# Amelie-Schreiber/ShapeMol

Hardware: AMD Instinct MI355X
Metric: molecules/sec (1000-step DDPM sample, batch 256) (higher is better)
Workload: dtype f32 (matrix operands split exactly into 3 x bf16 pieces = 24 bits, six piece products, fp32 accumulate); 1 GPU; BASELINE configs[1]: batch 256 MOSES-prior molecules (9-27 atoms) per GPU, 1000-step chain, fp32 results, k=8, synthetic shapes + hash-filled weights; besides the 5 warm-up steps an untimed 200-step chain runs first to reach the loaded clocks; batch_per_gpu=256, atoms_per_gpu=5541, total_atoms=5541, noise=device Philox, trajectories=kept in HBM, launch=hipGraph replay, parallelism=dp1 (whole batches per rank), ranks_seen=1

## Files before the change

### shapemol_amd/csrc/shapemol_hip.hip

```cpp
#include "../../include/shapemol_hip.h"
#include "sm_device.h"
#include "sm_edge.h"
#include "sm_edge_bf16.h"
#include "sm_edge16.h"
#include "sm_node.h"
#include "sm_node16.h"
#include "sm_edge_stream.h"
#include "sm_misc.h"
#include "sm_cfg.h"
#include "sm_guide_groups.h"
#include "sm_mesh.h"
#include <hip/hip_ext.h>

#include <algorithm>
#include <cmath>
#include <cstdio>
#include <cstring>
#include <map>
#include <string>
#include <type_traits>
#include <vector>

#include "sm_pack.h"
#include "sm_devmem.h"
// ... 82 lines not shown
    int num_cu = 256;
    CloudSet cs; MeshSet ms; DevList mem_cs, mem_ms;
    int2 *wg_table = nullptr; int64_t wg_table_cap = 0; DevList mem_wg;
    shapemol_sd_ctx *field_sd = nullptr; double field_lr = 0.0; int field_step = 0;
    float4 *m_within = nullptr; int *m_out = nullptr, *m_cnt = nullptr; int64_t m_cap = 0, m_cnt_cap = 0; DevList mem_mesh;
    int64_t m_flag_groups = 0;
    double cfg_w = 0.0, cfg_p = 0.0; int cfg_type = 0, cfg_has_bounds = 0; float cfg_lo[3] = {}, cfg_hi[3] = {};
    float *cfg_tr_pos_u = nullptr, *cfg_tr_v_u = nullptr;
    float *pred_pos_u = nullptr, *pred_v_u = nullptr;
    float *shape_zero = nullptr;
    float *cfg_stat = nullptr; double *cfg_part = nullptr; unsigned *cfg_hist = nullptr;
    CfgGroupSet cgs;
    int *cfg_mol_grp = nullptr; int2 *cfg_blk_tab = nullptr; double *cfg_gpart = nullptr; int64_t cfg_tab_stride = 0;
    int first_step = 0;
    int *pin_off = nullptr, *pin_atom = nullptr, *pin_nbr = nullptr; int64_t n_pins = 0; int pin_steps = 0, pin_k = 0; DevList mem_pins;
    bool prof_on = false;
    std::vector<ProfRec> prof;
    hipEvent_t cur_e0 = nullptr, cur_e1 = nullptr;
    hipGraphExec_t gexec = nullptr, gexec_u = nullptr;
    int64_t n_captures = 0;
    int64_t launch_rec[8] = {}, graph_rec[8] = {};
    int64_t node_rec[8] = {};
    int64_t x2h_out_rec[4] = {};
    struct GraphKey { int64_t N = 0, B = 0; Guide guide = Guide::None; int fold = 0, gfuse = 0;
                      int cfg = 0 ; double cfgv[9] = {};
                      int cfg_groups = 0;
                      uint64_t field_gen = 0; double field_lr = 0.0; int field_step = 0;
                      bool operator==(const GraphKey &o) const {
                          if (!(N == o.N && B == o.B && guide == o.guide && fold == o.fold && gfuse == o.gfuse && cfg == o.cfg &&
                                cfg_groups == o.cfg_groups && field_gen == o.field_gen && field_lr == o.field_lr &&
                                field_step == o.field_step)) return false;
                          for (int i = 0; i < 9; ++i) if (cfgv[i] != o.cfgv[i]) return false;
                          return true;
                      } } gkey{};
    hipStream_t gstream = nullptr; bool gstream_set = false;
    void drop_graphs() {
        if (!gexec && !gexec_u) return;
        if (!gstream_set || hipStreamSynchronize(gstream) != hipSuccess) hipDeviceSynchronize();
        if (gexec) { hipGraphExecDestroy(gexec); gexec = nullptr; }
        if (gexec_u) { hipGraphExecDestroy(gexec_u); gexec_u = nullptr; }
    }
    const float *P(size_t off) const { return d_img + off; }
};

namespace {

#define SMK(kern, grid, block, shm, stream, ...)                                                                    \
    do {                                                                                                             \
        if (c->prof_on) hipExtLaunchKernelGGL(kern, grid, block, shm, stream, c->cur_e0, c->cur_e1, 0, __VA_ARGS__); \
        else hipLaunchKernelGGL(kern, grid, block, shm, stream, __VA_ARGS__);                                        \
    } while (0)

// ... 65 lines not shown
    if (N <= c->capN && B <= c->capB) return 0;
    HIPCHK(hipSetDevice(c->device));
    HIPCHK(hipDeviceSynchronize());
    c->drop_graphs();
    const int64_t capN = std::max<int64_t>(N, c->capN), capB = std::max<int64_t>(B, c->capB);
    c->ws.release();
    c->capN = c->capB = 0; c->lastN = c->lastB = 0; c->last_h = c->last_x = nullptr;
    if (workspace_alloc(c, capN, capB)) { c->ws.release(); return 1; }
    c->capN = capN; c->capB = capB;
    return 0;
}

}

#include "sm_guide_host.h"

namespace {

constexpr int kVnFoldBytes = kVnFoldCap * 3 * 4 + 32 * 8;

template <int H>
lg::In launch_in(const shapemol_ctx *c, int n_atoms) {
    constexpr bool chain16_fits = Chain16Lds<H>::BYTES <= 2 * EdgeImage16<H, H / 16>::TOTAL * 4;
    return {c->opt, {kVnFoldCap, kStreamTPR, CHAIN_COLS, kGraphCap, kLin6Chunk, chain16_fits}, c->KP, c->num_cu, H, n_atoms};
}

#define ATTR(bytes, ...) HIPCHK(hipFuncSetAttribute((const void *)__VA_ARGS__, hipFuncAttributeMaxDynamicSharedMemorySize, (int)(bytes)))
template <int H, int K>
int set_edge_attr_k() {
    constexpr int NT = H / 16;
    constexpr int vn_tail = vn_red_doubles(12, H / 8) * 8 + 12 * 96 * 4;
    constexpr int fold = K <= 16 ? kVnFoldBytes : 0;
    constexpr int x16 = 2 * EdgeImage16<H, NT>::TOTAL * 4 + fold, h16 = (EdgeImage16<H, NT>::TOTAL + EdgeImage16<H, 1>::TOTAL) * 4 + vn_tail;
    ATTR(x16, edge16_kernel<H, K, false>); ATTR(x16, edge16_kernel<H, K, false, true>);
    ATTR(x16, edge16_loop_kernel<H, K, false>); ATTR(x16, edge16_loop_kernel<H, K, false, true>);
    ATTR(h16, edge16_kernel<H, K, true>); ATTR(h16, edge16_kernel<H, K, true, true>);
    ATTR(h16, edge16_loop_kernel<H, K, true>); ATTR(h16, edge16_loop_kernel<H, K, true, true>);
    ATTR((StreamMap<H, false>::O_TAIL * 4 + kVnFoldBytes), edge_stream_kernel<H, K, false>);
    ATTR((StreamMap<H, true>::O_TAIL * 4 + (NT + kStreamProducers) * 64 * 2 * 8), edge_stream_kernel<H, K, true>);
    if constexpr (K <= 16) {
        constexpr int xph = EdgePhaseImage<H, NT>::TOTAL * 4, hph = (EdgePhaseImage<H, NT>::TOTAL + EdgePhaseImage<H, 1>::TOTAL) * 4 + vn_tail;
        ATTR(x16, x2h_chain16_kernel<H, K>); ATTR(x16, x2h_chain16_kernel<H, K, true>);
        ATTR((EdgeBlob<H, false>::TOTAL * 4), edge_attention_kernel<H, K, false>); ATTR((EdgeBlob<H, true>::TOTAL * 4), edge_attention_kernel<H, K, true>);
        ATTR(xph, edge_fused_kernel<H, K, false, false>); ATTR(xph, edge_fused_kernel<H, K, false, true>);
        ATTR(hph, edge_fused_kernel<H, K, true, false>); ATTR(hph, edge_fused_kernel<H, K, true, true>);
    }
    return 0;
// ... 314 lines not shown
    c->tab_key = 0;
    LAUNCH("prep", SMK(prologue_tab_index_kernel, dim3((unsigned)((rows + 255) / 256)), dim3(256), 0, s, c->tab_v, c->tab_mol_of, c->tab_t_mol, c->tab_flag, T, C));
    const NodePrologueArgs pa = prologue_args<H>(c, c->tab_v, c->tab_mol_of, c->tab_t_mol, nullptr, c->etab, c->q_tab, c->pre_tab, (int)rows);
    if (launch_prologue<H>(c, s, pa, c->tab_flag)) return 1;
    c->tab_key = prologue_tab_key(c);
    return 0;
}

template <int H>
int run_score(shapemol_ctx *c, hipStream_t s, const ShapePrep &sp, const float *x_in, const int64_t *v_in, int64_t N, int64_t B,
              bool sampling, int t_first, float *out_pos, float *out_h, float *out_v, bool reuse_graph = false) {
    const shapemol_config &g = c->cfg;
    const int L = g.num_layers, hd = g.n_heads, C = g.num_classes, D = g.time_emb_dim, KP = c->KP;
    const int n = (int)N;
    AtomEmbArgs ae{c->P(c->dm.embw), c->P(c->dm.embb), v_in, c->mol_of, c->ttab, c->t_mol, sampling ? c->steps : nullptr,
                   c->steps + 1, c->bn_acc, c->h_a, n, H, C, D, t_first, L * kBnReplicas * 2 * hd + L};
    const int nlay = c->opt.stop_layer >= 0 ? std::min(c->opt.stop_layer, L) : L;
    const lg::In gi = launch_in<H>(c, n);
    const lg::StepForms sf = lg::step_forms(gi, sampling, c->n_pins > 0);
    if (sf.fused_prologue && c->opt.prologue_tab) {
        if (c->tab_key != prologue_tab_key(c)) return fail("run_score: the prologue tables are not built for this precision mode");
        PrologueTabArgs ta{c->etab, c->q_tab, c->pre_tab, c->tab_flag, v_in, c->mol_of, c->t_mol, ae.step_ptr, ae.step_cur, c->bn_acc,
                           sp.add0, c->h_a, c->q_x, c->pre0, c->status + ST_RANGE, n, C, g.num_timesteps, t_first, ae.bn_acc_len};
        LAUNCH("node_prologue", SMK(node_prologue_tab_kernel<H>, dim3((unsigned)((N * 16 + kProTabThreads - 1) / kProTabThreads)), dim3(kProTabThreads), 0, s, ta));
    } else if (sf.fused_prologue) {
        NodePrologueArgs pa = prologue_args<H>(c, v_in, c->mol_of, c->t_mol, sp.add0, c->h_a, c->q_x, c->pre0, n);
        pa.step_ptr = ae.step_ptr; pa.step_cur = ae.step_cur; pa.bn_acc = c->bn_acc; pa.bn_acc_len = ae.bn_acc_len; pa.t_first = t_first;
        if (nlay == 0) pa.n_lin_tiles = 0;
        pa.stamps = c->kstamp_sel == 5 ? c->kstamps : nullptr;
        if (launch_prologue<H>(c, s, pa)) return 1;
    } else {
        LAUNCH("embed", SMK(atom_embed_kernel, dim3((N * H + 255) / 256), dim3(256), 0, s, ae));
    }
    int64_t (&rec)[8] = c->launch_rec;
    std::fill(rec, rec + 8, 0);
    std::fill(c->node_rec, c->node_rec + 8, 0);
    std::fill(c->x2h_out_rec, c->x2h_out_rec + 4, 0);
    rec[0] = sampling; rec[1] = sf.graph_fused; rec[7] = c->num_cu;
    if (sf.stream && nlay > 0) { const lg::StreamGeom g = lg::stream_geom(gi); rec[5] = g.chunk; rec[6] = g.grid; }
    if (reuse_graph) {
    } else if (sf.graph_fused) {
        GraphArgs ga{x_in, c->mol_span, n, g.knn, KP, c->nbr, c->P(c->dm.ew.w1), c->P(c->dm.ew.b1), c->P(c->dm.ew.g), c->P(c->dm.ew.be),
                     c->P(c->dm.ew.w2), c->P(c->dm.ew.b2), c->ew, c->status + ST_SPAN, c->kstamp_sel == 4 ? c->kstamps : nullptr};
        const int apb = kGraphWaves * (KP >= 16 ? 1 : 16 / KP);
        DISPATCH_KP("graph", graph_kernel, (), dim3((n + apb - 1) / apb), dim3(kGraphWaves * 64), 0, s, ga);
    } else LAUNCH("knn", SMK(knn_kernel, dim3((N + 3) / 4), dim3(256), 0, s, x_in, c->mol_of, c->mol_off, n, g.knn, KP, c->nbr));
    if (sampling && c->n_pins > 0 && !reuse_graph)
        LAUNCH("knn", SMK(knn_pin_kernel, dim3(32), dim3(256), 0, s, c->pin_off, c->pin_steps, c->pin_atom, c->pin_nbr, c->pin_k, KP, c->steps + 1, n, c->nbr));
    EdgeWeightArgs ea{x_in, c->nbr, c->P(c->dm.ew.w1), c->P(c->dm.ew.b1), c->P(c->dm.ew.g), c->P(c->dm.ew.be),
                      c->P(c->dm.ew.w2), c->P(c->dm.ew.b2), c->ew, n * KP, KP};
    if (!sf.graph_fused && !reuse_graph) {
        const int tiles = (n * KP + 15) / 16;
        LAUNCH("edge_weight", SMK(edge_weight_kernel<H>, dim3((tiles + 3) / 4), dim3(256), 0, s, ea));
    }
    const float *cur_x = x_in;
    float *cur_h = c->h_a;
    constexpr int NT = H / 16;
    bool v_done = false;
    if (nlay > 0 && !sf.fused_prologue) {
        const DevLayer &D0 = c->dm.layer[0];
        if (launch_linear<H>(c, s, "node_pre", cur_h, c->P(D0.pre_x2h), c->P(D0.pre6_x2h), c->P(D0.pre16_x2h), sp.add0, 4 * H, c->pre0, 4 * H, 4 * NT, n,
                             c->kstamp_sel == 0 ? c->kstamps : nullptr)) return 1;
        if (launch_mlp2<H, 1>(c, s, "node_q", D0.q_x2h, cur_h, nullptr, NODE_LN_RELU, nullptr, c->q_x, H, H, n)) return 1;
    }
    double *stat_acc = c->bn_acc;
    if (c->bn_eval) {
// ... 112 lines not shown
        }
        cur_x = x_next;
    }
    c->last_h = cur_h; c->last_x = cur_x;
    if (nlay == 0 && out_pos) HIPCHK(hipMemcpyAsync(out_pos, x_in, N * 3 * sizeof(float), hipMemcpyDeviceToDevice, s));
    if (out_v && !v_done) {
        if (launch_mlp2<H, 1>(c, s, "v_head", c->dm.vhead, cur_h, nullptr, NODE_SSP, nullptr, out_v, C, C, n)) return 1;
    }
    return 0;
}

template <int H>
int run_ddpm(shapemol_ctx *c, hipStream_t s, int64_t N) {
    const shapemol_config &g = c->cfg;
    DdpmArgs a{};
    a.pred_pos = c->pred_pos; a.pred_v = c->pred_v; a.x_t = c->x_state; a.v_t = c->v_state; a.mol_of = c->mol_of;
    a.t_first = c->cfg.num_timesteps - 1;
    a.c0 = c->P(c->dm.tab[0]); a.ct = c->P(c->dm.tab[1]); a.logvar = c->P(c->dm.tab[2]); a.log_a = c->P(c->dm.tab[3]);
    a.log_1ma = c->P(c->dm.tab[4]); a.log_abar = c->P(c->dm.tab[5]); a.log_1mabar = c->P(c->dm.tab[6]);
    a.cp = c->chain_params; a.step_cur = c->steps + 1; a.step_ptr = c->steps;
    a.x_next = c->x_state; a.v_next = c->v_state;
    a.n_atoms = (int)N; a.C = g.num_classes;
    a.vf = c->ddpm_vf; c->ddpm_vf = DdpmFold{};
    const CfgArgs cfg = cfg_args(c, N);
    if (c->stamp_on) LAUNCH("stamp", SMK(clock_stamp_kernel, dim3(1), dim3(64), 0, s, c->stamps, c->steps + 1, 1024));
    if (g.num_classes <= 16) LAUNCH("ddpm", SMK(ddpm_step16_kernel, dim3((N * 16 + 255) / 256), dim3(256), 0, s, a, cfg));
    else LAUNCH("ddpm", SMK(ddpm_step_kernel<32>, dim3((N + 127) / 128), dim3(128), 0, s, a, cfg));
    return 0;
}

int check_cfg(const shapemol_config &g) {
    if (g.hidden_dim != 128 && g.hidden_dim != 32) return fail("hidden_dim must be 128 (or 32 for the reduced test model)");
    if (g.n_heads * 8 != g.hidden_dim) return fail("hidden_dim / n_heads must be 8");
    if (g.num_r_gaussian != 20) return fail("num_r_gaussian must be 20 (fixed RBF centres)");
    if (g.knn < 1 || g.knn > 32) return fail("knn must be in 1..32");
    if (g.shape_dim < 1 || g.shape_dim > 64 || g.shape_latent_dim < 4 || g.shape_latent_dim > 64 || (g.shape_latent_dim & 3))
        return fail("shape_dim must be 1..64, shape_latent_dim a multiple of 4 in 4..64");
    if (g.time_emb_dim < 4 || g.time_emb_dim > 16 || (g.time_emb_dim & 1)) return fail("time_emb_dim must be even, 4..16");
    if (g.num_classes < 2 || g.num_classes > 32) return fail("num_classes must be 2..32");
    if (g.num_layers < 1 || g.num_timesteps < 1) return fail("num_layers / num_timesteps must be positive");
    return 0;
}

template <typename F>
auto dispatch_h(const shapemol_ctx *c, F &&f) {
    return c->cfg.hidden_dim == 128 ? f(std::integral_constant<int, 128>{}) : f(std::integral_constant<int, 32>{});
}

}
// ... 65 lines not shown
        HIPCHK(c->mem_bn.alloc(&c->bn_run, 2 * count * sizeof(float)));
        HIPCHK(c->mem_bn.alloc(&c->bn_eval_acc, (size_t)L * kBnReplicas * 2 * hd * sizeof(double)));
    }
    HIPCHK(hipMemcpy(c->bn_run, h_mean, count * sizeof(float), hipMemcpyHostToDevice));
    HIPCHK(hipMemcpy(c->bn_run + count, h_var, count * sizeof(float), hipMemcpyHostToDevice));
    return 0;
}

int shapemol_reserve(shapemol_ctx *c, int64_t max_atoms, int64_t max_mols) {
    if (!c || max_atoms < 1 || max_mols < 1) return fail("shapemol_reserve: bad argument");
    return ensure_workspace(c, max_atoms, max_mols);
}

int shapemol_score(shapemol_ctx *c, const float *d_pos, const int64_t *d_v, const int64_t *d_batch, int64_t N,
                   int64_t B, const float *d_shape, const int64_t *d_t, float *out_pos, float *out_h, float *out_v,
                   void *stream) {
    if (!c || !d_pos || !d_v || !d_batch || !d_shape || !d_t || !out_pos || !out_v) return fail("shapemol_score: null argument");
    if (N < 1 || B < 1 || N > (1 << 27)) return fail("shapemol_score: n_atoms / n_mols out of range");
    HIPCHK(hipSetDevice(c->device));
    if (ensure_workspace(c, N, B)) return 1;
    hipStream_t s = (hipStream_t)stream;
    c->lastN = N; c->lastB = B;
    if (dispatch_h(c, [&](auto h) { return ensure_prologue_tables<h()>(c, s); })) return 1;
    HIPCHK(hipMemsetAsync(c->status, 0, 8 * sizeof(int), s));
    if (dispatch_h(c, [&](auto h) { return run_prep<h()>(c, s, d_batch, N, B, d_shape, c->prep[0]); })) return 1;
    LAUNCH("prep", SMK(t_convert_kernel, dim3((B + 255) / 256), dim3(256), 0, s, d_t, (int)B, c->cfg.num_timesteps, c->t_mol, c->status));
    LAUNCH("prep", SMK(v_check_kernel, dim3((N + 255) / 256), dim3(256), 0, s, d_v, (int)N, c->cfg.num_classes, c->status));
    return dispatch_h(c, [&](auto h) { return run_score<h()>(c, s, c->prep[0], d_pos, d_v, N, B, false, 0, out_pos, out_h, out_v); });
}

int shapemol_sample(shapemol_ctx *c, const float *d_init_pos, const int64_t *d_init_v, const int64_t *d_batch,
                    int64_t N, int64_t B, const float *d_shape, int32_t num_steps, const float *d_eps, const float *d_u,
                    uint64_t seed, const shapemol_traj *traj, float *out_pos, int64_t *out_v, int32_t use_graph, void *stream) {
    if (!c || !d_init_pos || !d_init_v || !d_batch || !d_shape || !out_pos || !out_v) return fail("shapemol_sample: null argument");
    if (N < 1 || B < 1 || N > (1 << 27)) return fail("shapemol_sample: n_atoms / n_mols out of range");
    if (num_steps < 1 || c->first_step + num_steps > c->cfg.num_timesteps) return fail("shapemol_sample: num_steps out of range");
    if ((d_eps == nullptr) != (d_u == nullptr)) return fail("shapemol_sample: d_eps and d_u must be given together");
    HIPCHK(hipSetDevice(c->device));
    if (ensure_workspace(c, N, B)) return 1;
    hipStream_t s = (hipStream_t)stream;
    c->lastN = N; c->lastB = B;
    if (dispatch_h(c, [&](auto h) { return ensure_prologue_tables<h()>(c, s); })) return 1;
    const int t_first = c->cfg.num_timesteps - 1;
    const Guide kind = chain_guide(c);
    const bool mesh = kind == Guide::Mesh, cfg = kind == Guide::Cfg;
    if (mesh && mesh_workspace(c, N, c->ms.groups)) return 1;
// ... 15 lines not shown
    if (cfg) {
        if (dispatch_h(c, [&](auto h) { return run_prep_shape<h()>(c, s, B, c->shape_zero, c->prep[1]); })) return 1;
        HIPCHK(hipMemsetAsync(c->cfg_hist, 0, (size_t)2 * kCfgHistWords * sizeof(unsigned), s));
        if (c->cgs.groups > 0) {
            const CfgArgs ca = cfg_args(c, N);
            HIPCHK(hipMemsetAsync(c->cgs.hist, 0, (size_t)c->cgs.groups * 2 * kCfgHistWords * sizeof(unsigned), s));
            LAUNCH("prep", SMK(cfg_groups_table_kernel, dim3(1), dim3(256), 0, s, d_batch, (int)N, ca.C, ca.n_groups, (int)B, ca.pf, c->cgs.rows,
                               c->cfg_mol_grp, c->cfg_blk_tab, ca.tab_stride, ca.blocks[0], ca.blocks[1]));
            c->cgs.stream = s; c->cgs.stream_set = true; c->cgs.last_groups = c->cgs.groups;
        }
    }
    LAUNCH("prep", SMK(v_check_kernel, dim3((N + 255) / 256), dim3(256), 0, s, d_init_v, (int)N, c->cfg.num_classes, c->status));
    {
        ChainParams cp{};
        cp.seed = seed; cp.eps = d_eps; cp.u = d_u; cp.step_base = c->first_step; cp.guide_draws = mesh ? c->ms.draws : c->cs.draws;
        if (traj) { cp.tr_pos = traj->pos_traj; cp.tr_v = traj->v_traj; cp.tr_v0 = traj->v0_traj; cp.tr_vt = traj->vt_traj;
                    cp.tr_pos_cond = traj->pos_cond_traj; cp.tr_v_cond = traj->v_cond_traj; }
        if (cfg && c->cgs.groups > 0) { cp.tr_pos_uncond = c->cgs.tr_pos_u; cp.tr_v_uncond = c->cgs.tr_v_u; }
        else if (cfg) { cp.tr_pos_uncond = c->cfg_tr_pos_u; cp.tr_v_uncond = c->cfg_tr_v_u; }
        LAUNCH("prep", SMK(set_chain_params_kernel, dim3(1), dim3(1), 0, s, c->chain_params, cp, c->steps));
    }
    HIPCHK(hipMemcpyAsync(c->x_state, d_init_pos, N * 3 * sizeof(float), hipMemcpyDeviceToDevice, s));
    HIPCHK(hipMemcpyAsync(c->v_state, d_init_v, N * sizeof(int64_t), hipMemcpyDeviceToDevice, s));
    auto one_step = [&]() -> int {
        if (dispatch_h(c, [&](auto h) { return run_score<h()>(c, s, c->prep[0], c->x_state, c->v_state, N, B, true, t_first, c->pred_pos, nullptr, c->pred_v); })) return 1;
        if (cfg) {
            if (dispatch_h(c, [&](auto h) { return run_score<h()>(c, s, c->prep[1], c->x_state, c->v_state, N, B, true, t_first, c->pred_pos_u, nullptr, c->pred_v_u, true); }) ||
                run_cfg_stats(c, s, cfg_args(c, N))) return 1;
        }
        if (enqueue_guidance(c, s, kind, c->pred_pos, N, c->steps + 1, t_first)) return 1;
        return dispatch_h(c, [&](auto h) { return run_ddpm<h()>(c, s, N); });
    };
    if (use_graph && !c->prof_on) {
        shapemol_ctx::GraphKey key{};
        const lg::StepForms sf = dispatch_h(c, [&](auto h) { return lg::step_forms(launch_in<h()>(c, (int)N), true, c->n_pins > 0); });
        key.N = N; key.B = B; key.guide = kind; key.fold = sf.fold; key.gfuse = sf.graph_fused;
        if (kind == Guide::Field) { key.field_gen = field_gen; key.field_lr = c->field_lr; key.field_step = c->field_step; }
        if (cfg && c->cgs.groups > 0) {
            key.cfg = 1 + c->cgs.type; key.cfg_groups = c->cgs.groups; key.cfgv[1] = c->cgs.p;
        } else if (cfg) {
            key.cfg = 1 + c->cfg_type;
            const double v[9] = {c->cfg_w, c->cfg_p, (double)c->cfg_has_bounds, c->cfg_lo[0], c->cfg_lo[1], c->cfg_lo[2], c->cfg_hi[0], c->cfg_hi[1], c->cfg_hi[2]};
            std::copy(v, v + 9, key.cfgv);
        }
        auto capture = [&](int n_steps, hipGraphExec_t *exec) -> int {
            hipGraph_t graph = nullptr;
            HIPCHK(hipStreamBeginCapture(s, hipStreamCaptureModeThreadLocal));
            int rc = 0;
            for (int i = 0; i < n_steps && !rc; ++i) rc = one_step();
            const hipError_t ce = hipStreamEndCapture(s, &graph);
            if (rc) { if (graph) hipGraphDestroy(graph); return 1; }
            if (ce != hipSuccess) return fail(std::string("hipStreamEndCapture: ") + hipGetErrorString(ce));
            const hipError_t ie = hipGraphInstantiate(exec, graph, nullptr, nullptr, 0);
            hipGraphDestroy(graph);
            if (ie != hipSuccess) { *exec = nullptr; return fail(std::string("hipGraphInstantiate: ") + hipGetErrorString(ie)); }
            ++c->n_captures;
            hipGraphUpload(*exec, s);
            return 0;
        };
// ... 41 lines not shown
        return 0;
    }
    if (k == "stop_layer") c->opt.stop_layer = (int)value;
    else if (k == "edge_bf16") {
        if (value < 0 || value > 3) return fail("edge_bf16 must be 0 (fp32 MFMA), 1 (exactly split bf16, phase kernels), 2 (exactly split bf16, streaming kernels) or 3 (two-piece f16)");
        if (value != 3 && value != 2 && c->KP > 16) return fail("k > 16 runs on the streaming (edge_bf16 = 2) or the two-piece f16 (edge_bf16 = 3) edge kernels");
        if (value == 3 && c->hid_max > 6.0e4f) return fail("edge_bf16 = 3: the edge MLPs' LayerNorm outputs may exceed the fp16 range for these weights");
        c->opt.edge_bf16 = (int)value;
    }
    else if (k == "edge_tiles") { if (value < -1 || value > 1) return fail("edge_tiles must be -1 (automatic), 0 (sliced one-job launches) or 1 (looping launch)"); c->opt.edge_tiles = (int)value; }
    else if (k == "node_f16") c->opt.node_f16 = value != 0;
    else if (k == "feat_f16") {
        if (value && (c->opt.edge_bf16 != 3 || !c->opt.node_f16)) return fail("feat_f16 = 1 needs the f16 kernels (edge_bf16 = 3, node_f16 = 1)");
        c->opt.feat_f16 = value != 0;
    }
    else if (k == "lin_fuse") c->opt.lin_fuse = value != 0;
    else if (k == "stream_whole_rounds") c->opt.stream_whole_rounds = value != 0;
    else if (k == "x2h_chain") c->opt.x2h_chain = value != 0;
    else if (k == "graph_fuse") c->opt.graph_fuse = value != 0;
    else if (k == "bn_eval") c->bn_eval = value != 0;
    else if (k == "ddpm_fold") c->opt.ddpm_fold = value != 0;
    else if (k == "vn_fold") c->opt.vn_fold = value != 0;
    else if (k == "prologue_tab") c->opt.prologue_tab = value != 0;
    else if (k == "lin_bf16") c->opt.lin_bf16 = (int)value;
    else if (k == "chain_bf16") c->opt.chain_bf16 = (int)value;
    else if (k == "vn_fuse") c->opt.vn_fuse = (int)value;
    else if (k == "node_levels") c->opt.node_levels = value != 0;
    else if (k == "x2h_out_fuse") { if (value < 0 || value > 2) return fail("x2h_out_fuse must be 0 (node_out6_kernel), 1 (x2h tail inside its boundary) or 2 (x2h tail always)"); c->opt.x2h_out_fuse = (int)value; }
    else if (k == "stream_chunk") { if (value < 0 || value > 4096) return fail("stream_chunk must be 0 (automatic) .. 4096"); c->opt.stream_chunk_opt = (int)value; }
    else if (k == "after_order") { if (value < 0 || value > 2) return fail("after_order must be 0 (follow-up jobs first), 1 (interleaved) or 2 (linear jobs first)"); c->opt.after_order = (int)value; }
    else if (k == "after_waves") { if (value < 1 || value > 16) return fail("after_waves must be 1..16"); c->opt.after_waves = (int)value; }
    else if (k == "after_lin_wgs") { if (value < 0 || value > 4096) return fail("after_lin_wgs must be 0 (automatic) .. 4096"); c->opt.after_lin_wgs = (int)value; }
    else if (k == "lin_waves") { if (value < 1 || value > 16) return fail("lin_waves must be 1..16"); c->opt.lin_waves = (int)value; }
    else if (k == "stamps") c->stamp_on = (int)value;
    else if (k == "kstamp_sel") c->kstamp_sel = (int)value;
    else if (k == "edge_waves") { if (value < 0 || value > 12) return fail("edge_waves must be 0 (automatic) .. 12"); c->opt.edge_threads = (int)value * 64; }
    else return fail("unknown option " + k);
    hipSetDevice(c->device);
    c->drop_graphs();
    return 0;
}

int64_t shapemol_debug_read(shapemol_ctx *c, const char *name, void *dst, size_t max_bytes) {
    if (!c || !name || !dst) { fail("shapemol_debug_read: null argument"); return -1; }
    const std::string k(name);
    const shapemol_config &g = c->cfg;
    const int64_t N = c->lastN;
    const void *src = nullptr; size_t bytes = 0;
    int64_t dims[8] = {N, c->lastB, c->KP, g.hidden_dim, g.n_heads, g.num_layers, c->capN, c->capB};
    if (k == "dims") { if (max_bytes < sizeof(dims)) return -1; std::memcpy(dst, dims, sizeof(dims)); return sizeof(dims); }
    if (k == "captures") { if (max_bytes < 8) return -1; std::memcpy(dst, &c->n_captures, 8); return 8; }
    if (k == "launch") { if (max_bytes < sizeof(c->launch_rec)) return -1; std::memcpy(dst, c->launch_rec, sizeof(c->launch_rec)); return sizeof(c->launch_rec); }
    if (k == "launch_x2h_out") { if (max_bytes < sizeof(c->x2h_out_rec)) return -1; std::memcpy(dst, c->x2h_out_rec, sizeof(c->x2h_out_rec)); return sizeof(c->x2h_out_rec); }
    if (k == "launch_node") { if (max_bytes < sizeof(c->node_rec)) return -1; std::memcpy(dst, c->node_rec, sizeof(c->node_rec)); return sizeof(c->node_rec); }
    if (k == "nbr") { src = c->nbr; bytes = N * c->KP * 4; }
    else if (k == "ew") { src = c->ew; bytes = N * c->KP * 4; }
    else if (k == "h") { src = c->last_h; bytes = N * g.hidden_dim * 4; }
    else if (k == "x") { src = c->last_x; bytes = N * 3 * 4; }
    else if (k == "h0") { src = c->h_a; bytes = N * g.hidden_dim * 4; }
    else if (k == "q_x") { src = c->q_x; bytes = N * g.hidden_dim * 4; }
    else if (k == "pre0") { src = c->pre0; bytes = N * 4 * g.hidden_dim * 4; }
    else if (k == "add0") { src = c->prep[0].add0; bytes = (size_t)c->lastB * 4 * g.hidden_dim * 4; }
    else if (k == "pre") { src = c->preAB; bytes = N * 8 * g.hidden_dim * 4; }
    else if (k == "q") { src = c->q_h; bytes = N * g.hidden_dim * 4; }
    else if (k == "att") { src = c->att; bytes = N * g.hidden_dim * 4; }
    else if (k == "o3") { src = c->o3; bytes = N * 48 * 4; }
    else if (k == "stamps") { src = c->stamps; bytes = 2048 * 8; }
    else if (k == "kstamps") { src = c->kstamps; bytes = (size_t)8 * 16 * 4096 * 8; }
    else if (k == "vn_err") { src = c->status + ST_VN_BARRIER; bytes = 4; }
    else if (k == "mesh_group_flags") { src = c->m_cnt ? c->m_cnt + 4 * c->m_cnt_cap : nullptr; bytes = (size_t)c->m_flag_groups * 4; }
    else if (k == "cfg_stat") { src = c->cfg_stat; bytes = 2 * 4; }
    else if (k == "cfg_group_stat") { src = c->cgs.last_groups > 0 ? c->cgs.stat : nullptr; bytes = (size_t)c->cgs.last_groups * 2 * 4; }
    else if (k == "bnstat") { src = c->bn_acc; bytes = (size_t)g.num_layers * kBnReplicas * 2 * g.n_heads * 8; }
    else { fail("shapemol_debug_read: unknown buffer " + k); return -1; }
    if (!src || bytes > max_bytes) { fail("shapemol_debug_read: buffer unavailable or destination too small"); return -1; }
    if (hipSetDevice(c->device) != hipSuccess || hipDeviceSynchronize() != hipSuccess ||
// ... 163 lines not shown
```

### shapemol_amd/csrc/sm_launch.h

```cpp
#pragma once
#include <algorithm>

namespace lg {

struct Options {
    int stop_layer = -1, edge_threads = 0 , lin_waves = 16, edge_bf16 = 2, lin_bf16 = 1, chain_bf16 = 1, vn_fuse = 2;
    int vn_fold = 1;
    int max_mol_atoms = 0;
    int stream_whole_rounds = 0;
    int lin_fuse = 0;
    int ddpm_fold = 1;
    int graph_fuse = 1;
    int x2h_chain = 1;
    int node_levels = 1;
    int x2h_out_fuse = 1;
    int stream_chunk_opt = 0;
    int after_order = 2;
    int after_waves = 16;
    int after_lin_wgs = 0;
    int node_f16 = 0;
    int feat_f16 = 0;
    int edge_tiles = -1;
    int prologue_tab = 1;
};

struct KernelConsts { int vn_fold_cap, stream_tpr, chain_cols, graph_cap, lin6_chunk; bool chain16_fits; };

struct In { Options o; KernelConsts k; int KP, num_cu, H, n_atoms; };

inline int cdiv(int a, int b) { return (a + b - 1) / b; }

struct Jobs { int apj, jobs; bool half; };
inline Jobs tile_jobs(int KP, int n_atoms) {
    const int apj = KP >= 16 ? 1 : 16 / KP;
    return {apj, KP > 16 ? 2 * n_atoms : cdiv(n_atoms, apj), KP > 16};
}

enum class Form { One, Loop, Sliced, Strided };
struct EdgeGeom { Form form; int apj, jobs, waves, grid, chunk, slice, atoms_per_wg; };

inline int edge_waves(const In &in, int jobs) {
    return in.o.edge_threads > 0 ? in.o.edge_threads / 64 : std::max(4, std::min(12, cdiv(jobs, in.num_cu)));
}
inline EdgeGeom one_job_geom(const In &in, int waves) {
    const Jobs j = tile_jobs(in.KP, in.n_atoms);
    const int grid = std::max(1, std::min(in.num_cu, cdiv(j.jobs, waves)));
    return {j.jobs <= grid * waves ? Form::One : Form::Strided, j.apj, j.jobs, waves, grid, waves, grid * waves, j.half ? 0 : waves * j.apj};
}

inline EdgeGeom edge_fp32_geom(const In &in) {
    const Jobs j = tile_jobs(in.KP, in.n_atoms);
// ... 68 lines not shown
    const int slots = in.num_cu * per_cu;
    g.n_fjobs = n_follow * g.n_pairs;
    g.tpg = 1;
    if (lin_tiles > 0) {
        const int ogroups = cdiv(lin_tiles, g.lw);
        const int lin_wgs = in.o.after_lin_wgs > 0 ? in.o.after_lin_wgs : std::max(slots - g.n_fjobs, slots / 2);
        g.tpg = std::max(1, cdiv(g.n_ct, std::max(1, lin_wgs / ogroups)));
        g.n_ljobs = ogroups * cdiv(g.n_ct, g.tpg);
    }
    g.lin_chunk = std::min(g.tpg, per_cu == 2 ? kAfterChunk : in.k.lin6_chunk);
    return g;
}

struct StepForms {
    bool fused_prologue;
    bool graph_fused;
    bool fold;
    bool f16, stream, phases;
    bool half_tiles;
    bool lin_fused;
    bool levels;
    bool out_fused;
    bool xc_fused;
};
inline StepForms step_forms(const In &in, bool sampling, bool pins) {
    const Options &o = in.o;
    const int KP = in.KP, m = o.max_mol_atoms;
    StepForms f{};
    f.fused_prologue = o.chain_bf16 && o.lin_bf16;
    f.graph_fused = sampling && o.graph_fuse && m > 0 && m <= in.k.graph_cap && KP <= 32 && !pins;
    f.f16 = o.edge_bf16 == 3; f.stream = o.edge_bf16 == 2; f.phases = o.edge_bf16 && KP <= 16;
    f.half_tiles = (f.f16 || f.stream) && KP > 16;
    f.lin_fused = o.chain_bf16 && o.lin_bf16 && o.node_f16 && o.lin_fuse;
    f.levels = o.node_levels && o.chain_bf16 && o.lin_bf16 && !o.node_f16 && !f.lin_fused;
    const StreamGeom sg = stream_geom(in);
    const EdgeGeom e16 = edge16_geom(in), xc = x2h_chain_geom(in);
    f.xc_fused = f.f16 && o.x2h_chain && KP <= 16 && o.chain_bf16 && o.node_f16 && !o.lin_fuse && o.edge_threads == 0 &&
                 xc.form == Form::One && xc.waves <= 12 && xc.atoms_per_wg <= in.k.chain_cols * 16 && in.k.chain16_fits;
    f.out_fused = f.stream && o.x2h_out_fuse && f.levels && KP <= 16 && (o.x2h_out_fuse == 2 || sg.atoms_per_wg <= 3 * in.k.chain_cols * 16);
    const int own = f.stream ? sg.atoms_per_wg : std::max(e16.atoms_per_wg, xc.atoms_per_wg);
    f.fold = sampling && o.vn_fold && (f.f16 || f.stream) && KP <= 16 && o.vn_fuse == 2 && m > 0 && (f.stream || o.edge_threads == 0) &&
             own + 2 * (m - 1) <= in.k.vn_fold_cap;
    return f;
}

}
```

### shapemol_amd/csrc/sm_misc.h

```cpp
#pragma once
#include "sm_device.h"
#include "sm_cfg.h"

enum StatusFlag { ST_VN_BARRIER = 0, ST_BATCH = 1, ST_ATOM_TYPE = 2, ST_TIME = 3, ST_RANGE = 4, ST_SPAN = 5, ST_MESH = 6 };

__global__ void mol_index_kernel(const int64_t *batch, int n, int n_mols, int *mol_of, int *mol_off, int *status) {
    const int i = blockIdx.x * blockDim.x + threadIdx.x;
    if (i >= n) return;
    const int64_t braw = batch[i], praw = i == 0 ? -1 : batch[i - 1];
    if (braw < 0 || braw >= n_mols || braw < praw) status[ST_BATCH] = 1;
    const int b = (int)min(max(braw, (int64_t)0), (int64_t)n_mols - 1);
    const int prev = (int)min(max(praw, (int64_t)-1), (int64_t)n_mols - 1);
    mol_of[i] = b;
    for (int m = prev + 1; m <= b; ++m) mol_off[m] = i;
    if (i == n - 1)
        for (int m = b + 1; m <= n_mols; ++m) mol_off[m] = n;
}

__global__ void mol_span_kernel(const int *mol_of, const int *mol_off, int n, int2 *span) {
    const int i = blockIdx.x * blockDim.x + threadIdx.x;
    if (i < n) span[i] = int2{mol_off[mol_of[i]], mol_off[mol_of[i] + 1]};
}

__global__ void t_convert_kernel(const int64_t *t, int n_mols, int n_timesteps, int *t_mol, int *status) {
// ... 214 lines not shown
    const float *te = a.ttab + (size_t)t * a.D;
    for (int k = 0; k < a.D; ++k) y += w[a.C + k] * te[k];
    a.h[idx] = y;
}

struct PrologueTabArgs {
    const float *etab, *q_tab, *pre_tab;
    const int *tab_flag;
    const int64_t *v;
    const int *mol_of;
    const int *t_mol;
    const int *step_ptr;
    int *step_cur;
    double *bn_acc;
    const float *add_mol;
    float *h_out, *q_out, *pre_out;
    int *range_flag;
    int n_atoms, C, T, t_first, bn_acc_len;
};

constexpr int kProTabThreads = 256;

template <int H>
__global__ void __launch_bounds__(kProTabThreads)
node_prologue_tab_kernel(PrologueTabArgs a) {
    constexpr int R = H / 64;
    static_assert(H % 64 == 0 || H == 32, "16 lanes x 16 bytes cover a row in whole passes");
    const int gid = blockIdx.x * kProTabThreads + threadIdx.x;
    const int step = a.step_ptr ? *a.step_ptr : 0;
    if (gid == 0) {
        if (a.step_ptr) *a.step_cur = step;
        if (*a.tab_flag) *a.range_flag = 1;
    }
    for (int i = gid; i < a.bn_acc_len; i += gridDim.x * kProTabThreads) a.bn_acc[i] = 0.0;
    const int atom = gid >> 4, ln = gid & 15;
    if (atom >= a.n_atoms) return;
    const int mol = a.mol_of[atom];
    const int t = min(max(a.step_ptr ? a.t_first - step : a.t_mol[mol], 0), a.T - 1);
    const int vi = min(max((int)a.v[atom], 0), a.C - 1);
    const size_t row = (size_t)t * a.C + vi;
    if constexpr (H == 32) {
        const int f = 4 * (ln & 7);
        const float *src = (ln < 8 ? a.etab : a.q_tab) + row * H + f;
        const float4 hq = ldg4(src);
        const float4 p0 = ldg4(a.pre_tab + row * 4 * H + 4 * ln), p1 = ldg4(a.pre_tab + row * 4 * H + 64 + 4 * ln);
        const float4 m0 = ldg4(a.add_mol + (size_t)mol * 4 * H + 4 * ln), m1 = ldg4(a.add_mol + (size_t)mol * 4 * H + 64 + 4 * ln);
        stg4((ln < 8 ? a.h_out : a.q_out) + (size_t)atom * H + f, hq);
        stg4(a.pre_out + (size_t)atom * 4 * H + 4 * ln, float4{p0.x + m0.x, p0.y + m0.y, p0.z + m0.z, p0.w + m0.w});
        stg4(a.pre_out + (size_t)atom * 4 * H + 64 + 4 * ln, float4{p1.x + m1.x, p1.y + m1.y, p1.z + m1.z, p1.w + m1.w});
    } else {
        float4 h[R], q[R], p[4 * R], m[4 * R];
#pragma unroll
        for (int r = 0; r < R; ++r) {
            h[r] = ldg4(a.etab + row * H + 64 * r + 4 * ln);
            q[r] = ldg4(a.q_tab + row * H + 64 * r + 4 * ln);
        }
#pragma unroll
        for (int r = 0; r < 4 * R; ++r) {
            p[r] = ldg4(a.pre_tab + row * 4 * H + 64 * r + 4 * ln);
            m[r] = ldg4(a.add_mol + (size_t)mol * 4 * H + 64 * r + 4 * ln);
        }
#pragma unroll
        for (int r = 0; r < R; ++r) {
            stg4(a.h_out + (size_t)atom * H + 64 * r + 4 * ln, h[r]);
            stg4(a.q_out + (size_t)atom * H + 64 * r + 4 * ln, q[r]);
        }
#pragma unroll
        for (int r = 0; r < 4 * R; ++r)
            stg4(a.pre_out + (size_t)atom * 4 * H + 64 * r + 4 * ln, float4{p[r].x + m[r].x, p[r].y + m[r].y, p[r].z + m[r].z, p[r].w + m[r].w});
    }
}

__global__ void prologue_tab_index_kernel(int64_t *v, int *mol_of, int *t_mol, int *flag, int T, int C) {
    const int i = blockIdx.x * blockDim.x + threadIdx.x;
    if (i == 0) *flag = 0;
    if (i < T) t_mol[i] = i;
    if (i < T * C) { v[i] = i % C; mol_of[i] = i / C; }
}

SM_DEV float dist2_rounded(float dx, float dy, float dz) {
#pragma clang fp contract(off)
    const float a = dx * dx, b = dy * dy, c = dz * dz;
    return (a + b) + c;
}

__global__ void knn_kernel(const float *x, const int *mol_of, const int *mol_off, int n_atoms, int k,
                           int kp, int *nbr) {
    const int lane = threadIdx.x & 63;
    const int i = blockIdx.x * (blockDim.x >> 6) + (threadIdx.x >> 6);
    if (i >= n_atoms) return;
    const int m = mol_of[i], s = mol_off[m], cnt = mol_off[m + 1] - s;
    const float xi = x[i * 3], yi = x[i * 3 + 1], zi = x[i * 3 + 2];
    const int deg = min(k, cnt - 1);
// ... 177 lines not shown
    }
    red[threadIdx.x][0] = o[0]; red[threadIdx.x][1] = o[1]; red[threadIdx.x][2] = o[2];
    __syncthreads();
    if (ok && c < 3) {
        float res = 0.f, att = 0.f;
        for (int h = 0; h < heads; ++h) res += red[la * heads + h][c];
        const float *ob = a.o3 + (size_t)i * 48;
        for (int r = 0; r < 16; ++r) att += ob[r * 3 + c];
        a.x_out[i * 3 + c] = a.x[i * 3 + c] + (att / heads + res / heads);
    }
}

constexpr int kGraphCap = 128;
constexpr int kGraphWaves = 8;
struct GraphArgs {
    const float *x;
    const int2 *mol_span;
    int n_atoms, k, kp;
    int *nbr;
    const float *w1, *b1, *g, *be, *w2, *b2;
    float *ew;
    int *span_flag;
    unsigned long long *stamps;
};
template <int H, int KP>
__global__ void __launch_bounds__(kGraphWaves * 64)
graph_kernel(GraphArgs a) {
    constexpr int NT = H / 16;
    constexpr int APW = KP >= 16 ? 1 : 16 / KP;
    constexpr int LPA = 64 / APW;
    constexpr int NQ = kGraphCap / LPA;
    constexpr int TPW = KP > 16 ? KP / 16 : 1;
    __shared__ float w1s[H * 20];
    __shared__ unsigned long long dkey[kGraphWaves][APW][kGraphCap];
    __shared__ float xs[kGraphWaves][APW][kGraphCap][3];
    __shared__ int row[kGraphWaves][APW * KP];
    __shared__ __attribute__((aligned(16))) float prm[4][H];
    const int lane = threadIdx.x & 63, wave = threadIdx.x >> 6;
    const int n = lane & 15, g = lane >> 4;
    const int sub = lane / LPA, l = lane % LPA;
    const int i_raw = (blockIdx.x * kGraphWaves + wave) * APW + sub;
    const bool valid = i_raw < a.n_atoms;
    const int i = valid ? i_raw : a.n_atoms - 1;
    SM_TICK(a.stamps, 0);
    const int2 span = a.mol_span[i];
    for (int idx = threadIdx.x; idx < H * 20; idx += kGraphWaves * 64) w1s[idx] = a.w1[idx];
    for (int idx = threadIdx.x; idx < 4 * H; idx += kGraphWaves * 64) {
        const int which = idx / H, f = idx % H;
        prm[which][f] = (which == 0 ? a.b1 : which == 1 ? a.g : which == 2 ? a.be : a.w2)[f];
    }
// ... 210 lines not shown
            const float m2 = fmaxf(lvt, l1_t);
            const float q2 = m2 + logf(expf(lvt - m2) + expf(l1_t - m2));
            un[c] = q1 + q2;
            umx = fmaxf(umx, un[c]);
        }
        float us = 0.f;
        for (int c = 0; c < C; ++c) us += expf(un[c] - umx);
        const float ulse = umx + logf(us);
        int best = 0;
        float bestv = -INFINITY;
        for (int c = 0; c < C; ++c) {
            const float lp = un[c] - ulse;
            if (a.tr_vt) a.tr_vt[so * C + c] = lp;
            const float gum = -logf(-logf(uu[c] + 1e-30f) + 1e-30f);
            const float sc = gum + lp;
            if (sc > bestv) { bestv = sc; best = c; }
        }
        a.v_next[i] = best;
        if (a.tr_v) a.tr_v[so] = best;
    }
    if (a.step_ptr && blockIdx.x == 0 && threadIdx.x == 0) *a.step_ptr = step + 1;
}

__global__ void __launch_bounds__(256) ddpm_step16_kernel(DdpmArgs aa, CfgArgs cfg) {
    struct : DdpmArgs, ChainParams {} a;
    static_cast<DdpmArgs &>(a) = aa;
    static_cast<ChainParams &>(a) = *aa.cp;
    const int gid = blockIdx.x * 256 + threadIdx.x;
    const int i_raw = gid >> 4, c = gid & 15;
    const int step = a.step_cur ? *a.step_cur : 0;
    const bool atom_ok = i_raw < a.n_atoms;
    const int i = atom_ok ? i_raw : a.n_atoms - 1;
    const int C = a.C;
    const bool cls = c < C;
    const int t = a.t_first - step;
    const size_t so = (size_t)(step - a.step_base) * a.n_atoms + i;
    float eps = 0.f, uu = 0.5f;
    if (a.eps) {
        if (c < 3) eps = a.eps[so * 3 + c];
        if (cls) uu = a.u[so * C + c];
    } else {
        Philox ph{(uint32_t)a.seed, (uint32_t)(a.seed >> 32)};
        uint32_t r[4];
        if (c < 3) {
            ph((uint32_t)i, (uint32_t)step, 0u, 0x5eedu, r);
            const float rad = sqrtf(-2.0f * logf(u01_open(c < 2 ? r[0] : r[2])));
            const float ang = 6.283185307179586f * u01_half(c < 2 ? r[1] : r[3]);
// ... 70 lines not shown
    }
    const float mx = seg_max<16>(lg);
    const float se = seg_sum<16>(cls ? expf(lg - mx) : 0.f);
    const float lv0 = lg - (mx + logf(se));
    const int tm1 = t > 0 ? t - 1 : 0;
    const float logC = logf((float)C);
    const float la_prev = a.log_abar[tm1], l1_prev = a.log_1mabar[tm1] - logC;
    const float la_t = a.log_a[t], l1_t = a.log_1ma[t] - logC;
    const int vt = (int)a.v_t[i];
    const float A1 = lv0 + la_prev;
    const float m1 = fmaxf(A1, l1_prev);
    const float q1 = m1 + logf(expf(A1 - m1) + expf(l1_prev - m1));
    const float lvt = (c == vt ? 0.f : -69.07755278982137f) + la_t;
    const float m2 = fmaxf(lvt, l1_t);
    const float q2 = m2 + logf(expf(lvt - m2) + expf(l1_t - m2));
    const float un = cls ? q1 + q2 : -INFINITY;
    const float umx = seg_max<16>(un);
    const float us = seg_sum<16>(cls ? expf(un - umx) : 0.f);
    const float lp = un - (umx + logf(us));
    const float sc = cls ? (-logf(-logf(uu + 1e-30f) + 1e-30f)) + lp : -INFINITY;
    const float best = seg_max<16>(sc);
    const float cand = (sc == best) ? (float)c : 99.f;
    const float win = -seg_max<16>(-cand);
    if (atom_ok && cls) {
        if (a.tr_v_cond && !cfg.on) a.tr_v_cond[so * C + c] = lg;
        if (a.tr_v0) a.tr_v0[so * C + c] = lv0;
        if (a.tr_vt) a.tr_vt[so * C + c] = lp;
    }
    if (atom_ok && c == 0) {
        a.v_next[i] = (int64_t)win;
        if (a.tr_v) a.tr_v[so] = (int64_t)win;
    }
    if (a.step_ptr && gid == 0) *a.step_ptr = step + 1;
}

__global__ void gumbel_argmax_kernel(const float *logits, const float *u, int n, int C, uint64_t seed, int64_t *out) {
    const int i = blockIdx.x * blockDim.x + threadIdx.x;
    if (i >= n) return;
    Philox ph{(uint32_t)seed, (uint32_t)(seed >> 32)};
    int best = 0;
    float bestv = -INFINITY;
    uint32_t r[4];
    for (int c = 0; c < C; ++c) {
        float uc;
        if (u) uc = u[(size_t)i * C + c];
        else { if ((c & 3) == 0) ph((uint32_t)i, 0xFFFFFFFFu, (uint32_t)(c >> 2), 0xca7u, r); uc = u01_half(r[c & 3]); }
// ... 84 lines not shown
```

Measured before the change: 395.9 molecules/s.

## Fold next-step node prologue table gather into the DDPM step kernel

The per-step node_prologue_tab kernel is removed from the sampling loop. Its table gather for the next step (using the freshly sampled class and t-1) now runs at the end of ddpm_step16_kernel, and its bn_acc zeroing and step_cur bookkeeping move into graph_kernel. A one-off prologue launch before the chain seeds the first step. This saves one kernel launch and its global round-trip per diffusion step, at the cost of extra work and registers in the ddpm and graph kernels and more complex cross-step state.

```diff
diff --git a/shapemol_amd/csrc/shapemol_hip.hip b/shapemol_amd/csrc/shapemol_hip.hip
--- a/shapemol_amd/csrc/shapemol_hip.hip
+++ b/shapemol_amd/csrc/shapemol_hip.hip
@@ -128,12 +128,14 @@
     int64_t launch_rec[8] = {}, graph_rec[8] = {};
     int64_t node_rec[8] = {};
     int64_t x2h_out_rec[4] = {};
-    struct GraphKey { int64_t N = 0, B = 0; Guide guide = Guide::None; int fold = 0, gfuse = 0;
+    int64_t prologue_rec[4] = {0, 0, -1, 0};
+    PrologueTabArgs ddpm_nxt{};
+    struct GraphKey { int64_t N = 0, B = 0; Guide guide = Guide::None; int fold = 0, gfuse = 0, pfold = 0;
                       int cfg = 0 ; double cfgv[9] = {};
                       int cfg_groups = 0;
                       uint64_t field_gen = 0; double field_lr = 0.0; int field_step = 0;
                       bool operator==(const GraphKey &o) const {
-                          if (!(N == o.N && B == o.B && guide == o.guide && fold == o.fold && gfuse == o.gfuse && cfg == o.cfg &&
+                          if (!(N == o.N && B == o.B && guide == o.guide && fold == o.fold && gfuse == o.gfuse && pfold == o.pfold && cfg == o.cfg &&
                                 cfg_groups == o.cfg_groups && field_gen == o.field_gen && field_lr == o.field_lr &&
                                 field_step == o.field_step)) return false;
                           for (int i = 0; i < 9; ++i) if (cfgv[i] != o.cfgv[i]) return false;
@@ -245,7 +247,8 @@
 template <int H>
 lg::In launch_in(const shapemol_ctx *c, int n_atoms) {
     constexpr bool chain16_fits = Chain16Lds<H>::BYTES <= 2 * EdgeImage16<H, H / 16>::TOTAL * 4;
-    return {c->opt, {kVnFoldCap, kStreamTPR, CHAIN_COLS, kGraphCap, kLin6Chunk, chain16_fits}, c->KP, c->num_cu, H, n_atoms};
+    return {c->opt, {kVnFoldCap, kStreamTPR, CHAIN_COLS, kGraphCap, kLin6Chunk, chain16_fits}, c->KP, c->num_cu, H, n_atoms,
+            c->cfg.num_classes, chain_guide(c) != Guide::None};
 }
 
 #define ATTR(bytes, ...) HIPCHK(hipFuncSetAttribute((const void *)__VA_ARGS__, hipFuncAttributeMaxDynamicSharedMemorySize, (int)(bytes)))
@@ -606,7 +609,8 @@
         if (c->tab_key != prologue_tab_key(c)) return fail("run_score: the prologue tables are not built for this precision mode");
         PrologueTabArgs ta{c->etab, c->q_tab, c->pre_tab, c->tab_flag, v_in, c->mol_of, c->t_mol, ae.step_ptr, ae.step_cur, c->bn_acc,
                            sp.add0, c->h_a, c->q_x, c->pre0, c->status + ST_RANGE, n, C, g.num_timesteps, t_first, ae.bn_acc_len};
-        LAUNCH("node_prologue", SMK(node_prologue_tab_kernel<H>, dim3((unsigned)((N * 16 + kProTabThreads - 1) / kProTabThreads)), dim3(kProTabThreads), 0, s, ta));
+        if (sf.prologue_folded) c->ddpm_nxt = ta;
+        else LAUNCH("node_prologue", SMK(node_prologue_tab_kernel<H>, dim3((unsigned)((N * 16 + kProTabThreads - 1) / kProTabThreads)), dim3(kProTabThreads), 0, s, ta));
     } else if (sf.fused_prologue) {
         NodePrologueArgs pa = prologue_args<H>(c, v_in, c->mol_of, c->t_mol, sp.add0, c->h_a, c->q_x, c->pre0, n);
         pa.step_ptr = ae.step_ptr; pa.step_cur = ae.step_cur; pa.bn_acc = c->bn_acc; pa.bn_acc_len = ae.bn_acc_len; pa.t_first = t_first;
@@ -626,6 +630,7 @@
     } else if (sf.graph_fused) {
         GraphArgs ga{x_in, c->mol_span, n, g.knn, KP, c->nbr, c->P(c->dm.ew.w1), c->P(c->dm.ew.b1), c->P(c->dm.ew.g), c->P(c->dm.ew.be),
                      c->P(c->dm.ew.w2), c->P(c->dm.ew.b2), c->ew, c->status + ST_SPAN, c->kstamp_sel == 4 ? c->kstamps : nullptr};
+        if (sf.prologue_folded) { ga.step_ptr = ae.step_ptr; ga.step_cur = ae.step_cur; ga.bn_acc = c->bn_acc; ga.bn_acc_len = ae.bn_acc_len; }
         const int apb = kGraphWaves * (KP >= 16 ? 1 : 16 / KP);
         DISPATCH_KP("graph", graph_kernel, (), dim3((n + apb - 1) / apb), dim3(kGraphWaves * 64), 0, s, ga);
     } else LAUNCH("knn", SMK(knn_kernel, dim3((N + 3) / 4), dim3(256), 0, s, x_in, c->mol_of, c->mol_off, n, g.knn, KP, c->nbr));
@@ -784,9 +789,11 @@
     a.x_next = c->x_state; a.v_next = c->v_state;
     a.n_atoms = (int)N; a.C = g.num_classes;
     a.vf = c->ddpm_vf; c->ddpm_vf = DdpmFold{};
+    const PrologueTabArgs nxt = c->ddpm_nxt; c->ddpm_nxt = PrologueTabArgs{};
     const CfgArgs cfg = cfg_args(c, N);
     if (c->stamp_on) LAUNCH("stamp", SMK(clock_stamp_kernel, dim3(1), dim3(64), 0, s, c->stamps, c->steps + 1, 1024));
-    if (g.num_classes <= 16) LAUNCH("ddpm", SMK(ddpm_step16_kernel, dim3((N * 16 + 255) / 256), dim3(256), 0, s, a, cfg));
+    if (g.num_classes <= 16 && nxt.pre_out) LAUNCH("ddpm", SMK(ddpm_step16_kernel<H>, dim3((N * 16 + 255) / 256), dim3(256), 0, s, a, cfg, nxt));
+    else if (g.num_classes <= 16) LAUNCH("ddpm", SMK(ddpm_step16_kernel<0>, dim3((N * 16 + 255) / 256), dim3(256), 0, s, a, cfg, nxt));
     else LAUNCH("ddpm", SMK(ddpm_step_kernel<32>, dim3((N + 127) / 128), dim3(128), 0, s, a, cfg));
     return 0;
 }
@@ -898,6 +905,7 @@
     hipStream_t s = (hipStream_t)stream;
     c->lastN = N; c->lastB = B;
     if (dispatch_h(c, [&](auto h) { return ensure_prologue_tables<h()>(c, s); })) return 1;
+    c->prologue_rec[0] = c->prologue_rec[1] = c->prologue_rec[3] = 0; c->prologue_rec[2] = -1;
     HIPCHK(hipMemsetAsync(c->status, 0, 8 * sizeof(int), s));
     if (dispatch_h(c, [&](auto h) { return run_prep<h()>(c, s, d_batch, N, B, d_shape, c->prep[0]); })) return 1;
     LAUNCH("prep", SMK(t_convert_kernel, dim3((B + 255) / 256), dim3(256), 0, s, d_t, (int)B, c->cfg.num_timesteps, c->t_mol, c->status));
@@ -959,6 +967,26 @@
     }
     HIPCHK(hipMemcpyAsync(c->x_state, d_init_pos, N * 3 * sizeof(float), hipMemcpyDeviceToDevice, s));
     HIPCHK(hipMemcpyAsync(c->v_state, d_init_v, N * sizeof(int64_t), hipMemcpyDeviceToDevice, s));
+    const lg::StepForms sf = dispatch_h(c, [&](auto h) { return lg::step_forms(launch_in<h()>(c, (int)N), true, c->n_pins > 0); });
+    if (sf.prologue_folded) {
+        if (c->tab_key != prologue_tab_key(c)) return fail("shapemol_sample: the prologue tables are not built for this precision mode");
+        const ShapePrep &sp = c->prep[0];
+        const int L = c->cfg.num_layers, hd = c->cfg.n_heads;
+        if (dispatch_h(c, [&](auto h) -> int {
+                constexpr int H = h();
+                PrologueTabArgs ta{c->etab, c->q_tab, c->pre_tab, c->tab_flag, c->v_state, c->mol_of, c->t_mol, c->steps, c->steps + 1, c->bn_acc,
+                                   sp.add0, c->h_a, c->q_x, c->pre0, c->status + ST_RANGE, (int)N, c->cfg.num_classes, c->cfg.num_timesteps, t_first,
+                                   L * kBnReplicas * 2 * hd + L};
+                LAUNCH("prep", SMK(node_prologue_tab_kernel<H>, dim3((unsigned)((N * 16 + kProTabThreads - 1) / kProTabThreads)), dim3(kProTabThreads), 0, s, ta));
+                return 0;
+            })) return 1;
+    }
+    {
+        const int t_last = t_first - (c->first_step + num_steps - 1);
+        c->prologue_rec[0] = sf.prologue_folded; c->prologue_rec[1] = sf.prologue_folded;
+        c->prologue_rec[2] = !sf.prologue_folded ? -1 : (t_last > 0 ? t_last - 1 : (num_steps >= 2 ? 0 : -1));
+        c->prologue_rec[3] = 0;
+    }
     auto one_step = [&]() -> int {
         if (dispatch_h(c, [&](auto h) { return run_score<h()>(c, s, c->prep[0], c->x_state, c->v_state, N, B, true, t_first, c->pred_pos, nullptr, c->pred_v); })) return 1;
         if (cfg) {
@@ -970,8 +998,7 @@
     };
     if (use_graph && !c->prof_on) {
         shapemol_ctx::GraphKey key{};
-        const lg::StepForms sf = dispatch_h(c, [&](auto h) { return lg::step_forms(launch_in<h()>(c, (int)N), true, c->n_pins > 0); });
-        key.N = N; key.B = B; key.guide = kind; key.fold = sf.fold; key.gfuse = sf.graph_fused;
+        key.N = N; key.B = B; key.guide = kind; key.fold = sf.fold; key.gfuse = sf.graph_fused; key.pfold = sf.prologue_folded;
         if (kind == Guide::Field) { key.field_gen = field_gen; key.field_lr = c->field_lr; key.field_step = c->field_step; }
         if (cfg && c->cgs.groups > 0) {
             key.cfg = 1 + c->cgs.type; key.cfg_groups = c->cgs.groups; key.cfgv[1] = c->cgs.p;
@@ -1059,6 +1086,7 @@
     else if (k == "ddpm_fold") c->opt.ddpm_fold = value != 0;
     else if (k == "vn_fold") c->opt.vn_fold = value != 0;
     else if (k == "prologue_tab") c->opt.prologue_tab = value != 0;
+    else if (k == "prologue_fold") c->opt.prologue_fold = value != 0;
     else if (k == "lin_bf16") c->opt.lin_bf16 = (int)value;
     else if (k == "chain_bf16") c->opt.chain_bf16 = (int)value;
     else if (k == "vn_fuse") c->opt.vn_fuse = (int)value;
@@ -1089,6 +1117,7 @@
     if (k == "captures") { if (max_bytes < 8) return -1; std::memcpy(dst, &c->n_captures, 8); return 8; }
     if (k == "launch") { if (max_bytes < sizeof(c->launch_rec)) return -1; std::memcpy(dst, c->launch_rec, sizeof(c->launch_rec)); return sizeof(c->launch_rec); }
     if (k == "launch_x2h_out") { if (max_bytes < sizeof(c->x2h_out_rec)) return -1; std::memcpy(dst, c->x2h_out_rec, sizeof(c->x2h_out_rec)); return sizeof(c->x2h_out_rec); }
+    if (k == "launch_prologue") { if (max_bytes < sizeof(c->prologue_rec)) return -1; std::memcpy(dst, c->prologue_rec, sizeof(c->prologue_rec)); return sizeof(c->prologue_rec); }
     if (k == "launch_node") { if (max_bytes < sizeof(c->node_rec)) return -1; std::memcpy(dst, c->node_rec, sizeof(c->node_rec)); return sizeof(c->node_rec); }
     if (k == "nbr") { src = c->nbr; bytes = N * c->KP * 4; }
     else if (k == "ew") { src = c->ew; bytes = N * c->KP * 4; }
diff --git a/shapemol_amd/csrc/sm_launch.h b/shapemol_amd/csrc/sm_launch.h
--- a/shapemol_amd/csrc/sm_launch.h
+++ b/shapemol_amd/csrc/sm_launch.h
@@ -22,11 +22,12 @@
     int feat_f16 = 0;
     int edge_tiles = -1;
     int prologue_tab = 1;
+    int prologue_fold = 1;
 };
 
 struct KernelConsts { int vn_fold_cap, stream_tpr, chain_cols, graph_cap, lin6_chunk; bool chain16_fits; };
 
-struct In { Options o; KernelConsts k; int KP, num_cu, H, n_atoms; };
+struct In { Options o; KernelConsts k; int KP, num_cu, H, n_atoms; int num_classes = 0; bool guided = false; };
 
 inline int cdiv(int a, int b) { return (a + b - 1) / b; }
 
@@ -141,6 +142,7 @@
     bool levels;
     bool out_fused;
     bool xc_fused;
+    bool prologue_folded;
 };
 inline StepForms step_forms(const In &in, bool sampling, bool pins) {
     const Options &o = in.o;
@@ -160,6 +162,8 @@
     const int own = f.stream ? sg.atoms_per_wg : std::max(e16.atoms_per_wg, xc.atoms_per_wg);
     f.fold = sampling && o.vn_fold && (f.f16 || f.stream) && KP <= 16 && o.vn_fuse == 2 && m > 0 && (f.stream || o.edge_threads == 0) &&
              own + 2 * (m - 1) <= in.k.vn_fold_cap;
+    f.prologue_folded = sampling && f.fused_prologue && o.prologue_tab && o.prologue_fold && f.graph_fused && in.num_classes >= 1 &&
+                        in.num_classes <= 16 && !in.guided && !pins;
     return f;
 }
 
diff --git a/shapemol_amd/csrc/sm_misc.h b/shapemol_amd/csrc/sm_misc.h
--- a/shapemol_amd/csrc/sm_misc.h
+++ b/shapemol_amd/csrc/sm_misc.h
@@ -260,22 +260,12 @@
 constexpr int kProTabThreads = 256;
 
 template <int H>
-__global__ void __launch_bounds__(kProTabThreads)
-node_prologue_tab_kernel(PrologueTabArgs a) {
+SM_DEV void prologue_tab_gather(const PrologueTabArgs &a, int atom, int ln, int t_raw, int v_raw) {
     constexpr int R = H / 64;
     static_assert(H % 64 == 0 || H == 32, "16 lanes x 16 bytes cover a row in whole passes");
-    const int gid = blockIdx.x * kProTabThreads + threadIdx.x;
-    const int step = a.step_ptr ? *a.step_ptr : 0;
-    if (gid == 0) {
-        if (a.step_ptr) *a.step_cur = step;
-        if (*a.tab_flag) *a.range_flag = 1;
-    }
-    for (int i = gid; i < a.bn_acc_len; i += gridDim.x * kProTabThreads) a.bn_acc[i] = 0.0;
-    const int atom = gid >> 4, ln = gid & 15;
-    if (atom >= a.n_atoms) return;
     const int mol = a.mol_of[atom];
-    const int t = min(max(a.step_ptr ? a.t_first - step : a.t_mol[mol], 0), a.T - 1);
-    const int vi = min(max((int)a.v[atom], 0), a.C - 1);
+    const int t = min(max(t_raw, 0), a.T - 1);
+    const int vi = min(max(v_raw, 0), a.C - 1);
     const size_t row = (size_t)t * a.C + vi;
     if constexpr (H == 32) {
         const int f = 4 * (ln & 7);
@@ -307,6 +297,21 @@
         for (int r = 0; r < 4 * R; ++r)
             stg4(a.pre_out + (size_t)atom * 4 * H + 64 * r + 4 * ln, float4{p[r].x + m[r].x, p[r].y + m[r].y, p[r].z + m[r].z, p[r].w + m[r].w});
     }
+}
+
+template <int H>
+__global__ void __launch_bounds__(kProTabThreads)
+node_prologue_tab_kernel(PrologueTabArgs a) {
+    const int gid = blockIdx.x * kProTabThreads + threadIdx.x;
+    const int step = a.step_ptr ? *a.step_ptr : 0;
+    if (gid == 0) {
+        if (a.step_ptr) *a.step_cur = step;
+        if (*a.tab_flag) *a.range_flag = 1;
+    }
+    for (int i = gid; i < a.bn_acc_len; i += gridDim.x * kProTabThreads) a.bn_acc[i] = 0.0;
+    const int atom = gid >> 4, ln = gid & 15;
+    if (atom >= a.n_atoms) return;
+    prologue_tab_gather<H>(a, atom, ln, a.step_ptr ? a.t_first - step : a.t_mol[a.mol_of[atom]], (int)a.v[atom]);
 }
 
 __global__ void prologue_tab_index_kernel(int64_t *v, int *mol_of, int *t_mol, int *flag, int T, int C) {
@@ -530,10 +535,16 @@
     float *ew;
     int *span_flag;
     unsigned long long *stamps;
+    const int *step_ptr; int *step_cur; double *bn_acc; int bn_acc_len;
 };
 template <int H, int KP>
 __global__ void __launch_bounds__(kGraphWaves * 64)
 graph_kernel(GraphArgs a) {
+    if (a.bn_acc) {
+        const int gid = blockIdx.x * (kGraphWaves * 64) + threadIdx.x;
+        if (gid == 0) *a.step_cur = *a.step_ptr;
+        for (int i = gid; i < a.bn_acc_len; i += gridDim.x * (kGraphWaves * 64)) a.bn_acc[i] = 0.0;
+    }
     constexpr int NT = H / 16;
     constexpr int APW = KP >= 16 ? 1 : 16 / KP;
     constexpr int LPA = 64 / APW;
@@ -790,7 +801,8 @@
     if (a.step_ptr && blockIdx.x == 0 && threadIdx.x == 0) *a.step_ptr = step + 1;
 }
 
-__global__ void __launch_bounds__(256) ddpm_step16_kernel(DdpmArgs aa, CfgArgs cfg) {
+template <int PH>
+__global__ void __launch_bounds__(256) ddpm_step16_kernel(DdpmArgs aa, CfgArgs cfg, PrologueTabArgs nxt) {
     struct : DdpmArgs, ChainParams {} a;
     static_cast<DdpmArgs &>(a) = aa;
     static_cast<ChainParams &>(a) = *aa.cp;
@@ -907,6 +919,12 @@
     const float best = seg_max<16>(sc);
     const float cand = (sc == best) ? (float)c : 99.f;
     const float win = -seg_max<16>(-cand);
+    if constexpr (PH > 0) {
+        if (nxt.pre_out && t > 0) {
+            if (gid == 0 && *nxt.tab_flag) *nxt.range_flag = 1;
+            if (atom_ok) prologue_tab_gather<PH>(nxt, i, c, t - 1, (int)win);
+        }
+    }
     if (atom_ok && cls) {
         if (a.tr_v_cond && !cfg.on) a.tr_v_cond[so * C + c] = lg;
         if (a.tr_v0) a.tr_v0[so * C + c] = lv0;
```

After: 397.8 molecules/s, median of 6. About the same (+0.5%).
